# vedantsawal/Cost-and-Carbon-Aware-Kubernetes-Autoscaler

Measured on AMD Instinct MI355X. Metric: policy-evaluated cluster-steps/sec, higher is better.
Workload: dtype int32+int64+f64; 1 GPU; config2: 1e5 clusters x 1 deployment x 1440 one-minute steps, HPA + peak/off-peak, 16-type catalog; scenarios_per_gpu=100000, steps_per_rollout=1440, mode=trajectory, schedule=lane-skewed (single deployment), trace_layout=wave-tiled [wave][T][lanes] (built by the first rollout), parallelism=scenario-sharded x1

## Files before the change

cost-and-carbon-aware-kubernetes-autoscaler_amd/csrc/d1_common.h:

```cpp
#pragma once
#include <hip/hip_runtime.h>
#include <stdint.h>

#include "../../include/ccka.h"
#include "kparams.h"

namespace ccka {
namespace {

constexpr int WAVE = 64;

__device__ __forceinline__ int capbit1(int c) { return c == 0 ? CCKA_CAP_SPOT : CCKA_CAP_OD; }

template <class V>
__device__ __forceinline__ V opq(V v) {
  asm volatile("" : "+s"(v));
  return v;
}
#define GLOBAL_AS __attribute__((address_space(1)))
template <class V>
__device__ __forceinline__ GLOBAL_AS V* opq_ptr(V* v) {
  uint64_t x = (uint64_t)v;
  asm volatile("" : "+s"(x));
  return (GLOBAL_AS V*)x;
}

__device__ __forceinline__ int wmask(int window_s) {
  int m = 0;
#pragma unroll
  for (int k = 0; k < CCKA_HIST; ++k) m |= ((k + 1) * CCKA_STEP_SECONDS < window_s) ? (1 << k) : 0;
  return m;
}

template <int W = 4>
__device__ __forceinline__ void ring_push(uint32_t* r, int v) {
#pragma unroll
  for (int w = W - 1; w > 0; --w) r[w] = __builtin_amdgcn_alignbit(r[w], r[w - 1], 16);
  r[0] = (r[0] << 16) | ((uint32_t)v & 0xFFFFu);
}
template <int W>
__device__ __forceinline__ void ring_push4(uint32_t* r, int v) {
#pragma unroll
  for (int w = W - 1; w > 1; --w) r[w] = r[w - 2];
  r[1] = r[0] = ((uint32_t)v & 0xFFFFu) * 0x10001u;
}

typedef short short2v __attribute__((ext_vector_type(2)));
__device__ __forceinline__ short2v as_s2(uint32_t x) { return __builtin_bit_cast(short2v, x); }
__device__ __forceinline__ uint32_t bfi(uint32_t m, uint32_t a, uint32_t b) { return (m & a) | (~m & b); }

__device__ __forceinline__ int fdiv_nb(int a, int b, float rb, bool& bad) {
  int q = (int)((float)a * rb);
  const int r = (int)((uint32_t)a - (uint32_t)q * (uint32_t)b);
  q += (r >= b ? 1 : 0) - (r < 0 ? 1 : 0);
  bad = bad || (uint32_t)q >= (1u << 20) || (uint32_t)b >= (1u << 30);
  return q;
}

constexpr int D1_NOSTORE = 0x7FFFFFF0;
__device__ __forceinline__ void d1_store_rec(__amdgpu_buffer_rsrc_t r, int voff, const int4& v) {
  typedef int i32x4 __attribute__((ext_vector_type(4)));
  const i32x4 x = {v.x, v.y, v.z, v.w};
  __builtin_amdgcn_raw_buffer_store_b128(x, r, voff, 0, 0);
}

#define CONST_AS __attribute__((address_space(4)))
__device__ __forceinline__ int2 d1_tload(const GLOBAL_AS int2* ptr) {
  const uint64_t a = (uint64_t)ptr;
  const int alo = (int)(uint32_t)a, ahi = (int)(uint32_t)(a >> 32);
  const int me = (int)(threadIdx.x & (WAVE - 1));
  uint64_t m = __ballot(1);
  int ox = 0, oy = 0;
  while (m) {
    int l[4];
#pragma unroll
    for (int k = 0; k < 4; ++k) {
      l[k] = m ? __ffsll((long long)m) - 1 : l[0];
      m &= m - 1;
    }
    uint64_t v[4];
#pragma unroll
    for (int k = 0; k < 4; ++k) {
      const uint64_t ak = (uint64_t)(uint32_t)__builtin_amdgcn_readlane(alo, l[k]) |
                          (uint64_t)(uint32_t)__builtin_amdgcn_readlane(ahi, l[k]) << 32;
      v[k] = *(const CONST_AS uint64_t*)ak;
    }
#pragma unroll
    for (int k = 0; k < 4; ++k) {
      ox = me == l[k] ? (int)(uint32_t)v[k] : ox;
      oy = me == l[k] ? (int)(uint32_t)(v[k] >> 32) : oy;
    }
  }
  return make_int2(ox, oy);
}

}
}
```

cost-and-carbon-aware-kubernetes-autoscaler_amd/csrc/rollout_d1.hip:

```cpp
#include <hip/hip_runtime.h>
#include <stdint.h>

#include "../../include/ccka.h"
#include "d1_common.h"
#include "kparams.h"

#pragma clang fp contract(off)

namespace ccka {

namespace {

struct Best {
  double s;
  int k;
  int info;
  int price;
};

__device__ __forceinline__ bool better(double s2, int k2, double s, int k) {
  return s2 < s || (s2 == s && k2 < k);
}

__device__ __forceinline__ void take_if_better(Best& a, const Best& b) {
// ... 187 lines not shown
          bool G3 = false, bool KEDA = false>
__global__ void __launch_bounds__(256, OCC) rollout_d1_kernel(D1Params p) {
  static_assert(NSUB == 1 || (NSUB == 4 && BDEF), "15 s sync: lean default path");
  static_assert(!KEDA || (BDEF && NSUB == 1 && !DRIFT), "KEDA: default behavior, one decision per step");
  static_assert(HE == 8 || (HE == 4 && NSUB == 1 && BDEF), "4-record ring: default behavior, one decision per step");
  static_assert(!G3 || (DRIFT && MAXP == 2), "G3: the DRIFT instantiation, two pools");
  constexpr int HW = NSUB == 1 ? HE / 2 : 10;
  constexpr int JR = NSUB == 1 ? HE : 5;
  uint64_t st_acc[12] = {0, 0, 0, 0, 0, 0, 0, 0, 0, 0, 0, 0};
  uint64_t st_last = STAMPS ? __builtin_amdgcn_s_memtime() : 0;
  extern __shared__ __attribute__((aligned(16))) int4 s_acc[];
  for (int x = threadIdx.x; x < p.K; x += blockDim.x) {
    const long long idle = p.acc[x * 3 + 0];
    s_acc[x] = make_int4((int)(idle & 0xffffffffLL), (int)(idle >> 32), (int)p.acc[x * 3 + 1], (int)p.acc[x * 3 + 2]);
  }
  const bool ldt = p.lds_tab;
  const uint32_t tab_off = ((uint32_t)p.K * 16u + 255u) / 256u * 256u + (blockDim.x / WAVE) * (uint32_t)D1_RING_BYTES;
  const int n_pr = p.R * 24 * p.K * p.Z * 2;
  const int n_pr8 = (n_pr + 1) & ~1;
  int* const s_price = reinterpret_cast<int*>(reinterpret_cast<char*>(s_acc) + tab_off);
  double* const s_ci = reinterpret_cast<double*>(s_price + n_pr8);
  int* const s_jtab = reinterpret_cast<int*>(s_ci + p.R * 24);
  if (ldt) {
    for (int x = threadIdx.x; x < n_pr; x += blockDim.x) s_price[x] = p.price[x];
    for (int x = threadIdx.x; x < p.R * 24; x += blockDim.x) s_ci[x] = p.ci_gpwmin[x];
    for (int x = threadIdx.x; x < p.R * 24 * p.NZI * 3; x += blockDim.x) s_jtab[x] = p.jtab[x];
  }
  __syncthreads();
  const int lane = threadIdx.x & (WAVE - 1);
  const int64_t wv = (int64_t)xcd_block(blockIdx.x, gridDim.x) * (blockDim.x / WAVE) + (threadIdx.x / WAVE);
  const int64_t i = wv * p.lpw + lane;
  if (lane >= p.lpw || i >= p.N) return;

  const int r = p.region ? (int)p.region[i] : 0;
  const int target = KEDA ? 1 : (p.target ? (int)p.target[i] : p.target0);
  const int mx = KEDA ? opq(p.k_max) : (p.maxr ? (int)p.maxr[i] : p.maxr0);
  const int dwin = (!KEDA && p.down_stab) ? (int)p.down_stab[i] : p.dstab0;
  const int nd = min(NSUB == 1 ? __popc(wmask(dwin)) : (dwin > 15 ? (dwin - 1) / 15 : 0), 2 * HW);
  const int dnmask = NSUB == 1 ? wmask(dwin) : 0;
  const int reset_ca = p.reset_ca ? (int)p.reset_ca[i] : p.reset_ca0;
  const int pswitch = p.pswitch ? (int)p.pswitch[i] : p.pswitch0;
  const int wi = p.wci ? (int)p.wci[i] : 0;
  const uint32_t capsel = p.cap_sel ? (uint32_t)p.cap_sel[i] : (uint32_t)p.capsel0;
  const int minr = KEDA ? max(opq(p.k_min), 1) : opq(p.minr), req = opq(p.req_cpu), limit = opq(p.limit);
  const int kthr = KEDA ? opq(p.k_thr) : 1, kact = KEDA ? opq(p.k_act) : 0, kcds = KEDA ? opq(p.k_cds) : 0;
  const bool kmin0 = KEDA && opq(p.k_min) == 0;
  const float rkthr = __builtin_amdgcn_rcpf((float)kthr);
  int ulo = max(0, (int)floor(p.tol_lo * (double)target) - 2);
  while ((double)ulo / (double)target < p.tol_lo) ++ulo;
  int uhi = (int)floor(p.tol_hi * (double)target) + 2;
  while ((double)uhi / (double)target > p.tol_hi) --uhi;
  const float rtarget = __builtin_amdgcn_rcpf((float)target);

  const int NP = opq(p.NP), NZI = opq(p.NZI), NW = opq(p.NW), JT = opq(p.JT);
  const int maxn = opq(p.maxn), ablate = CCKA_ABLATE_BUILD ? opq(p.ablate) : 0, pdb_member = opq(p.pdb_member);
  const int pdb_pct = opq(p.pdb_pct), slo_util = opq(p.slo_util), delay = opq(p.delay);
  const int base_nodes = opq(p.base_nodes), base_type = opq(p.base_type);
  const int K = opq(p.K), Z = opq(p.Z), T = opq(p.T);
  const int ps = opq(p.peak_start) % 1440, pe = opq(p.peak_end) % 1440;
  const int ps_raw = opq(p.peak_start), pe_raw = opq(p.peak_end);
  const int sm0 = opq(p.start_minute) % 1440;
  const long long base_nw = opq(p.base_nw);
  const GLOBAL_AS int32_t* const price = opq_ptr(p.price);
  const GLOBAL_AS double* const ci_gpwmin = opq_ptr(p.ci_gpwmin);
  const GLOBAL_AS int2* const table = opq_ptr(p.table);
  const GLOBAL_AS int2* const table2 = opq_ptr(p.table2);
  const int drift_on = opq(p.drift_on), replace = opq(p.replace), multi = G3 ? opq(p.multi) : 0;
  const GLOBAL_AS int32_t* const jtab = opq_ptr(p.jtab);
  GLOBAL_AS int4* const traj = opq_ptr(reinterpret_cast<int4*>(p.traj));
  const D1Rule rup = [&] { if constexpr (BDEF) return d1_default_rule(true); else return opq_rule(p.up); }();
  const D1Rule rdn = [&] { if constexpr (BDEF) return d1_default_rule(false); else return opq_rule(p.dn); }();
  int budget[MAXP];
#pragma unroll
  for (int q = 0; q < MAXP; ++q) budget[q] = opq(p.budget[q]);

  int ppol[MAXP], pcas[MAXP], pzi[MAXP], pJ[MAXP];
  uint32_t pcm[MAXP], pmask[MAXP];
#pragma unroll
  for (int q = 0; q < MAXP; ++q) {
    ppol[q] = 0; pcas[q] = 0; pzi[q] = -1; pcm[q] = 0; pJ[q] = 0; pmask[q] = 0;
    if (q < NP) {
#pragma unroll
      for (int s = 0; s < 2; ++s) {
        const D1Patch& x = p.patch[q][s];
        if (x.policy) ppol[q] = x.policy;
        if (x.cas >= 0) pcas[q] = s == 1 ? (reset_ca + CCKA_STEP_SECONDS - 1) / CCKA_STEP_SECONDS : x.cas;
        if (x.zi >= 0) pzi[q] = x.zi;
        if (x.cm) pcm[q] = (uint32_t)x.cm;
      }
    }
  }

  auto cas_of = [&](uint32_t info) {
    const int m1 = -(int)(info >> 13 & 1u), m2 = -(int)(info >> 14 & 1u);
    const int lo = pcas[0] ^ ((pcas[0] ^ pcas[MAXP > 1 ? 1 : 0]) & m1);
    if constexpr (MAXP <= 2) {
      return lo;
    } else {
      const int hi = pcas[2] ^ ((pcas[2] ^ pcas[3]) & m1);
      return lo ^ ((lo ^ hi) & m2);
    }
  };
  auto casc = [](int c) { return min(c, 0xFFFF); };

  uint32_t sinfo[MAXN];
  int sready[MAXN], slc[MAXN], scas[MAXN], spods[MAXN], sprice[MAXN], scap[MAXN];
  uint32_t sdyn[MAXN];
  int salloc[MAXN];
  int sallocr[MAXN];
#pragma unroll
  for (int n = 0; n < MAXN; ++n) {
    sinfo[n] = 0; sready[n] = 0; slc[n] = 0; scas[n] = 0; spods[n] = 0; sprice[n] = 0; scap[n] = 0;
    sdyn[n] = 0; salloc[n] = 0; sallocr[n] = 0;
  }
  uint32_t used = 0, rdy = 0, cmask = 0;
  auto dyn_of = [&](int n) -> uint32_t {
    if constexpr (G3) return (uint32_t)s_acc[sinfo[n] & 1023u].z;
    else return sdyn[n];
  };
  auto alloc_of = [&](int n) -> int {
    if constexpr (G3) return s_acc[sinfo[n] & 1023u].w;
    else return salloc[n];
  };
  constexpr bool kAllocR = NSUB == 1 && !G3;
  auto alloc_ready = [&](int n) -> uint32_t {
    if constexpr (kAllocR) return (uint32_t)sallocr[n];
    else return (rdy >> n & 1u) ? (uint32_t)alloc_of(n) : 0u;
  };
  auto cas_slot = [&](int n) -> int {
    if constexpr (G3) return casc(cas_of(sinfo[n]));
    else return scas[n];
  };
  uint32_t dmask = 0, srcm = 0, repm = 0;
  auto taint = [&]() -> uint32_t { return DRIFT ? (srcm | repm) : 0u; };
  auto od_slots = [&]() {
    uint32_t m = 0;
#pragma unroll
    for (int n = MAXN - 1; n >= 0; --n) m = 2 * m + (sinfo[n] >> 12 & 1u);
    return m & used;
  };
  const uint32_t slot_mask = maxn >= 32 ? 0xFFFFFFFFu : ((1u << maxn) - 1u);

  int replicas = p.replicas0, placed = 0, rpods = 0;
  uint32_t hdn[HW], hup[4], hdel[4] = {0, 0, 0, 0};
  uint32_t dn16[HW];
#pragma unroll
  for (int w = 0; w < 4; ++w) hup[w] = 0x7FFF7FFFu;
#pragma unroll
  for (int w = 0; w < HW; ++w) {
    hdn[w] = 0x80008000u;
    dn16[w] = (2 * w < nd ? 0xFFFFu : 0u) | (2 * w + 1 < nd ? 0xFFFF0000u : 0u);
  }
  int next_ready = 0x7fffffff, nsp = 0, nod = 0;
  int kcd = kcds, q_klo = 0, q_khi = -1, kb_cur = -1;
  bool q_kcd = false;
  bool k_act_step = false;
  auto keda_band = [&](int cur) {
    if (!KEDA || cur == kb_cur) return;
    kb_cur = cur;
    if (cur <= 0) { q_klo = 0; q_khi = -1; return; }
    const double D = (double)kthr * (double)cur;
    long long lo = max((long long)floor(p.tol_lo * D) - 2, -1LL);
    while ((double)lo / D < p.tol_lo) ++lo;
    long long hi = (long long)floor(p.tol_hi * D) + 2;
    while ((double)hi / D > p.tol_hi) --hi;
    q_klo = (int)min(lo, 0x7fffffffLL);
    q_khi = (int)min(hi, 0x7ffffffeLL);
  };
  keda_band(p.replicas0);
  int Ffree = 0;
  int minscap = 0x7fffffff;
  int profile = -1, hour = -1;
  long long cost = 0, burn = 0, base_price = 0;
  int pend_min = 0;
  long long energy_nw = 0, e_hour = 0, Isum = 0;
  double gco2 = 0.0, ci_min = 0.0;
  int slo = 0, nmin_spot = 0, nmin_od = 0, launches = 0, deletions = 0, peak_nodes = 0;
  uint32_t last_choice = 0xFFFFFFFFu, hash = 2166136261u;

  unsigned long long Ssum = 0;
  float Rmax = 0.f;
  float q_rbd = 0.f, q_rbc = 0.f, q_rbp = 0.f;
  bool q_peak = false;
  int q_rcap = 0;
  int q_hold = -0x40000000;
  (void)dnmask;
  const int wl = NSUB == 1 ? nd : max(0, (nd - (NSUB - 1)) / NSUB);
  const int wr = NSUB == 1 ? nd : (nd + NSUB - 1) / NSUB;
  int q_ulim = 0, q_pge = 0, q_slo = 0, q_usat = 0, q_w0 = 0, q_w1 = 0, q_pendv = 0, q_nodes = 0;
  float q_hbp = 0.f;
  uint32_t usum = 0;
  bool q_met = false;

  auto refresh_J = [&](int rh) {
#pragma unroll
    for (int q = 0; q < MAXP; ++q) {
      const uint32_t cm = pcm[q] & capsel;
      const int64_t ji = ((int64_t)rh * NZI + pzi[q]) * 3 + (cm - 1);
      pJ[q] = (q < NP && cm && pzi[q] >= 0) ? (ldt ? s_jtab[ji] : jtab[ji]) : 0;
    }
  };

  struct HpaOut {
    int util, proposal, desired;
    bool ran, hpa_path;
  };
  auto behave = [&](int proposal, int cur) -> int {
    int upr = proposal, dnr = proposal;
    if (rup.stab_mask) {
      short2v a = as_s2(bfi((uint32_t)rup.stab16[0], hup[0], 0x7FFF7FFFu));
#pragma unroll
      for (int w = 1; w < 4; ++w)
        a = __builtin_elementwise_min(a, as_s2(bfi((uint32_t)rup.stab16[w], hup[w], 0x7FFF7FFFu)));
      upr = min(upr, min((int)a.x, (int)a.y));
    }
    {
      short2v a = as_s2(bfi(dn16[0], hdn[0], 0x80008000u));
#pragma unroll
      for (int w = 1; w < HW; ++w) a = __builtin_elementwise_max(a, as_s2(bfi(dn16[w], hdn[w], 0x80008000u)));
      dnr = max(dnr, max((int)a.x, (int)a.y));
    }
    const int rc = min(max(cur, upr), dnr);
    int lo = minr, hi = mx;
    if constexpr (BDEF) {
      hi = rc > cur ? min(hi, max(2 * cur, cur + 4)) : hi;
      lo = rc < cur ? max(lo, 0) : lo;
    } else {
      if (proposal != cur) {
        if (rc > cur) hi = min(hi, max(rate_limit1(rup, true, cur, hdel), cur));
        else if (rc < cur) lo = max(lo, min(rate_limit1(rdn, false, cur, hdel), cur));
      }
    }
    return rc < lo ? lo : (rc > hi ? hi : rc);
  };
  auto hpa_eval = [&](int L, int cur, int ready, float rbd, float rbc) -> HpaOut {
    HpaOut o;
    const bool metric = cur <= mx && cur >= minr && ready > 0 && !(cur == 0 && minr != 0);
    int util = 0, proposal = cur;
    {
      const int rcapv = ready * limit;
      const int usage = (limit > 0 && rcapv < L) ? rcapv : L;
      const int a = usage * 100;
      const int dreq = ready * req;
      const int dcur = cur * req;
      bool slow = usage < 0 || usage > 21474836;
      util = fdiv_nb(a, dreq, rbd, slow);
      int nu = 0;
      if (cur > ready) nu = fdiv_nb(a, dcur, rbc, slow);
      if (__builtin_expect(metric && slow, 0))
        util = (int)(((long long)usage * 100) / ((long long)ready * req));
      const bool unready_up = cur > ready && util > target;
      int u = util, base = ready;
// ... 121 lines not shown
  }();
  const int32_t* lp = p.load_w ? p.load_w + wtb * T + lane
                               : p.load + (p.trace_mod > 0 ? (p.first_id + i) % p.trace_mod : i);
  const long long lsl = opq(p.load_w ? (long long)p.lpw : (long long)p.NL);
  const uint32_t ring_off = (uint32_t)__builtin_amdgcn_readfirstlane(
      (int)(((uint32_t)p.K * 16u + 255u) / 256u * 256u + (threadIdx.x / WAVE) * (uint32_t)D1_RING_BYTES));
  const uint32_t ring_lds = (uint32_t)(uintptr_t)s_acc + ring_off;
  const int* const ring = reinterpret_cast<const int*>(reinterpret_cast<const char*>(s_acc) + ring_off);
  constexpr int rsw = WAVE, rbn = D1_RB;
  auto rrow = [&](int x) { return x & (D1_RB - 1); };
  auto ridx = [&](int r) { return r * rsw + lane; };
  auto rnext = [&](int r, int q) { return (r + q) & (D1_RB - 1); };
  int tf = 0;
  int tfr = 0;
  const int32_t* lpf = lp;
  auto tf_adv = [&]() {
    ++tf;
    ++tfr;
    if (tfr == rbn) tfr = 0;
    lpf += lsl;
  };
  {
    const int n0 = min(T, D1_VMN + 4 * D1_S);
    while (tf < n0) {
      d1_dma_row(lpf, (uint32_t)__builtin_amdgcn_readfirstlane((int)(ring_lds + (uint32_t)tfr * (uint32_t)(rsw * 4))));
      tf_adv();
    }
    d1_wait_all();
  }
  int t_rdy = tf;
  bool pf_ok = false;
  bool qadv = true;
  int Lpf[D1_S];
#pragma unroll
  for (int q = 0; q < D1_S; ++q) Lpf[q] = 0;
  const int64_t w0 = wtb;
  const int wlanes = (int)min((int64_t)p.lpw, p.N - w0);
  const __amdgpu_buffer_rsrc_t trs = __builtin_amdgcn_make_buffer_rsrc(
      traj ? (void*)(reinterpret_cast<int4*>(p.traj) + w0 * T) : (void*)p.load, 0, traj ? wlanes * T * 16 : 0,
      0x00020000);
  const int lb = lane * T * 16;

  for (int it = 0;; ++it) {
    const bool live = t < T;
    if (__ballot(live) == 0) break;
    d1_wait_rows();
    t_rdy = max(t_rdy, tf - D1_VMN);
    const uint64_t sb = __ballot(stall);
    if constexpr (STAMPS) st_acc[9] += 1;
    if (sb != 0 && (it % D1_K == D1_K - 1 || !qadv)) {
      __builtin_amdgcn_s_setprio(0);
      if constexpr (STAMPS) { st_acc[10] += 1; st_acc[11] += __popcll(sb); }
      const bool ev = stall;
      int L = 0, minute = 0, rh = 0, pd = 0, step_last_type = 0xFFFF;
      int4 rec;
      uint32_t flags = 0;
      bool g_acted = false, hchg = false, jchg = false;
      uint32_t emp_e = 0, weou_e = 0;
      HpaOut hp{};
      if (ev) {
        stall = false;
        const int tr = rrow(t);
        L = ring[ridx(tr)];
        if constexpr (BDEF) {
          const int kq = min(t - tq, wr);
          if (kq > 0) {
            const int cur16 = min(replicas, D1_REC_SAT);
            int us[JR], rv[JR];
            bool anylow = false;
#pragma unroll
            for (int j = 0; j < JR; ++j) {
              us[j] = KEDA ? ring[ridx(rnext(tr, rbn - 1 - j))] : min(ring[ridx(rnext(tr, rbn - 1 - j))], q_rcap);
              rv[j] = q_met ? cur16 : (int)0x8000;
              anylow |= (j < kq) & q_met & (us[j] < q_pge);
            }
            if (KEDA && anylow) {
#pragma unroll
              for (int j = 0; j < JR; ++j) {
                bool sl = false;
                const bool low = (j < kq) & q_met & (us[j] < q_pge);
                const int q = fdiv_nb(max(us[j], 0), kthr, rkthr, sl);
                rv[j] = low ? min(q + (q * kthr != us[j] ? 1 : 0), D1_REC_SAT) : rv[j];
              }
            } else if (anylow) {
              const int dreq = rpods * req;
              const float rbd = __builtin_amdgcn_rcpf((float)dreq);
              bool anyex = false;
#pragma unroll
              for (int j = 0; j < JR; ++j) {
                bool sl = false;
                const bool low = (j < kq) & q_met & (us[j] < q_pge);
                const int util = fdiv_nb(us[j] * 100, dreq, rbd, sl);
                const int x = (int)__umul24((uint32_t)util, (uint32_t)rpods);
                const int q = fdiv_nb(x, target, rtarget, sl);
                const bool ex = x == q * target;
                anyex |= low & ex;
                rv[j] = low ? min(q + (ex ? 0 : 1), D1_REC_SAT) : rv[j];
                us[j] = (low & ex) ? util : -1;
              }
              if (__builtin_expect(anyex, 0)) {
#pragma unroll
                for (int j = 0; j < JR; ++j)
                  if (us[j] >= 0)
                    rv[j] = min((int)ceil(((double)us[j] / (double)target) * (double)rpods), D1_REC_SAT);
              }
            }
#pragma unroll
            for (int j = JR - 1; j >= 0; --j)
              if (j < kq) {
                if constexpr (NSUB == 1) ring_push<HW>(hdn, rv[j]);
                else ring_push4<HW>(hdn, rv[j]);
              }
          }
        }
        flush(t);
        minute = (sm0 + t) % 1440;
        const int h = minute / 60;
        rh = r * 24 + h;
        if (h != hour) {
          if (hour >= 0) {
            gco2 += (double)e_hour * (ci_min * 1e-9);
            energy_nw += e_hour;
          }
          e_hour = 0;
          hour = h;
          hchg = true;
        }
      }
      D1_STAMP(2);
      if (ev) {
        if (t >= next_ready) {
          next_ready = 0x7fffffff;
#pragma unroll
          for (int n = 0; n < MAXN; ++n) {
            if ((used & ~rdy) >> n & 1u) {
              if (sready[n] <= t) {
                rdy |= 1u << n;
                rpods += spods[n];
                sallocr[n] = salloc[n];
                if ((cmask & ~taint()) >> n & 1u) Ffree += scap[n] - spods[n];
              }
              else next_ready = min(next_ready, sready[n]);
            }
          }
        }
        const bool in_win = ps_raw <= pe_raw ? (minute >= ps_raw && minute < pe_raw)
                                             : (minute >= ps_raw || minute < pe_raw);
        const bool peak = pswitch && in_win;
        const int prof = peak ? CCKA_PROFILE_PEAK : CCKA_PROFILE_OFFPEAK;
        if (peak) flags |= 1u;
        q_peak = peak;
        if (prof != profile) {
          profile = prof;
          int pold[MAXP];
#pragma unroll
          for (int q = 0; q < MAXP; ++q) pold[q] = pcas[q];
#pragma unroll
          for (int q = 0; q < MAXP; ++q) {
            if (q >= NP) break;
            const D1Patch& x = p.patch[q][prof + 1];
            if (x.policy) ppol[q] = x.policy;
            if (x.cas >= 0) pcas[q] = x.cas;
            if (x.zi >= 0) pzi[q] = x.zi;
            if (x.cm) pcm[q] = (uint32_t)x.cm;
          }
#pragma unroll
          for (int n = 0; n < MAXN; ++n)
            if (used >> n & 1u) {
              const int c = casc(cas_of(sinfo[n]));
              if constexpr (G3) {
                const int m1 = -(int)(sinfo[n] >> 13 & 1u);
                const int o = pold[0] ^ ((pold[0] ^ pold[MAXP > 1 ? 1 : 0]) & m1);
                slc[n] += c - casc(o);
              } else {
                slc[n] += c - scas[n];
              }
              scas[n] = c;
            }
          jchg = true;
          if (DRIFT && drift_on) {
            uint32_t dm = 0;
#pragma unroll
            for (int n = 0; n < MAXN; ++n) {
              const uint32_t x = sinfo[n];
              uint32_t zm = 0, cm = 0;
#pragma unroll
              for (int q = 0; q < MAXP; ++q)
                if ((int)(x >> 13 & 3u) == q) { zm = pzi[q] >= 0 ? p.zml[pzi[q]] : 0u; cm = pcm[q]; }
              const bool drifted = !(zm >> (x >> 10 & 3u) & 1u) || !(cm & capbit1((int)(x >> 12 & 1u)));
              dm |= ((used >> n & 1u) && drifted ? 1u : 0u) << n;
            }
            dmask = dm;
          }
        }

      }
      D1_STAMP(3);
      if (ev) {
#pragma unroll
        for (int sub = 0; sub < NSUB; ++sub) {
          const int cur = replicas;
          if constexpr (KEDA) hp = keda_eval(L, cur, t);
          else
            hp = hpa_eval(L, cur, rpods, __builtin_amdgcn_rcpf((float)(rpods * req)),
                          __builtin_amdgcn_rcpf((float)(cur * req)));
          hpa_commit(hp, cur);
          replicas = hp.desired;
        }

        if (placed > replicas) {
          int excess = placed - replicas;
          placed = replicas;
#pragma unroll
          for (int pass = 0; pass < 2; ++pass) {
            const uint32_t m = pass == 0 ? (used & ~rdy) : rdy;
            if (!m || excess <= 0) continue;
            int removed = 0, removed_c = 0;
#pragma unroll
            for (int n = MAXN - 1; n >= 0; --n) {
              const int k = (m >> n & 1u) ? min(spods[n], excess) : 0;
              spods[n] -= k;
              excess -= k;
              removed += k;
              if (pass == 1) removed_c += ((cmask & ~taint()) >> n & 1u) ? k : 0;
              slc[n] = k > 0 ? t + cas_slot(n) : slc[n];
            }
            if (pass == 1) { rpods -= removed; Ffree += removed_c; }
          }
        }
        pd = replicas - placed;
        if (pd > 0) {
#pragma unroll
          for (int pass = 0; pass < 2; ++pass) {
            const uint32_t m = (pass == 0 ? rdy : (used & ~rdy)) & cmask & ~taint();
            if (!m || pd <= 0) continue;
            int added = 0;
#pragma unroll
            for (int n = 0; n < MAXN; ++n) {
              const int fr = (m >> n & 1u) ? scap[n] - spods[n] : 0;
              const int k = min(fr, pd);
              spods[n] += k;
              pd -= k;
              added += k;
              slc[n] = k > 0 ? t + cas_slot(n) : slc[n];
            }
            placed += added;
            if (pass == 0) { rpods += added; Ffree -= added; }
          }
        }
      }
      D1_STAMP(4);
      if (ev) {
        if (hchg) {
          const int64_t toff = (int64_t)rh * K * Z * 2;
          const GLOBAL_AS int32_t* tile = price + toff;
          const int* stile = s_price + toff;
          ci_min = ldt ? s_ci[rh] : ci_gpwmin[rh];
          base_price = (long long)base_nodes * (ldt ? stile[(base_type * Z) * 2 + 1] : tile[(base_type * Z) * 2 + 1]);
          burn = 0;
          int np[MAXN];
#pragma unroll
          for (int n = 0; n < MAXN; ++n) {
            const uint32_t x = sinfo[n];
            const int e = ((int)(x & 1023u) * Z + (int)(x >> 10 & 3u)) * 2 + (int)(x >> 12 & 1u);
            np[n] = ldt ? stile[e] : tile[e];
          }
#pragma unroll
          for (int n = 0; n < MAXN; ++n) {
            if (used >> n & 1u) {
              sprice[n] = np[n];
              burn += np[n];
            }
          }
        }
        if (hchg || jchg) refresh_J(rh);
        {
          uint32_t fm = ~used & slot_mask;
          if (pd > 0 && fm && !ablated(ablate, 2)) {
            int q = -1, J = 0, zq = 0, cq = 0;
            uint32_t cm = 0;
#pragma unroll
            for (int qq = MAXP - 1; qq >= 0; --qq) {
              const uint32_t c = pcm[qq] & capsel;
              if (qq < NP && c && pJ[qq] > 0) { q = qq; J = pJ[qq]; cm = c; zq = pzi[qq]; cq = pcas[qq]; }
            }
            if (q >= 0) {
              const GLOBAL_AS int2* row = table + ((((int64_t)rh * NZI + zq) * 3 + (cm - 1)) * NW + wi) * JT;
              while (pd > 0 && fm) {
                const int slot = __ffs((int)fm) - 1;
                fm &= fm - 1;
                const int k = min(J, pd);
                const int2 e = d1_tload(row + k);
                const int info = e.y, price = e.x;
                const int bk = info & 1023, bz = info >> 10 & 3, bc = info >> 12 & 1, cap1 = info >> 16;
                const int rs = t + delay;
                const int4 ac = s_acc[bk];
#pragma unroll
                for (int n = 0; n < MAXN; ++n) {
                  if (n == slot) {
                    sinfo[n] = (uint32_t)(bk | bz << 10 | bc << 12 | q << 13);
                    sready[n] = rs;
                    slc[n] = t + casc(cq);
                    scas[n] = casc(cq);
                    spods[n] = k;
                    sprice[n] = price;
                    scap[n] = cap1;
                    sdyn[n] = (uint32_t)ac.z;
                    salloc[n] = ac.w;
                    sallocr[n] = delay == 0 ? ac.w : 0;
                  }
                }
                const uint32_t bit = 1u << slot;
                used |= bit;
                if (capbit1(bc) & capsel) cmask |= bit;
#pragma unroll
                for (int qq = 0; qq < MAXP; ++qq) if (qq == q) pmask[qq] |= bit;
                placed += k;
                minscap = min(minscap, cap1);
                Isum += ((long long)ac.y << 32) | (unsigned)ac.x;
                if (delay == 0) {
                  rdy |= bit;
                  rpods += k;
                  if (cmask & bit) Ffree += cap1 - k;
                }
                else next_ready = min(next_ready, rs);
                if (bc == 0) nsp++; else nod++;
                burn += price;
                launches++;
                last_choice = (uint32_t)bk | (uint32_t)bz << 12 | (uint32_t)bc << 14 | (uint32_t)q << 16;
                hash = (hash ^ last_choice) * 16777619u;
                step_last_type = bk;
                flags |= 2u;
                pd -= k;
              }
            }
          }
        }

      }
      D1_STAMP(5);
      if (ev) {
        uint32_t elig = 0, emp = 0;
#pragma unroll
        for (int n = MAXN - 1; n >= 0; --n) {
          elig = 2 * elig + (slc[n] <= t ? 1u : 0u);
          emp = 2 * emp + (spods[n] == 0 ? 1u : 0u);
        }
        elig &= rdy;
        emp &= used;
        uint32_t weou = 0;
#pragma unroll
        for (int q = 0; q < MAXP; ++q)
          if (q < NP && ppol[q] == CCKA_WHEN_EMPTY_OR_UNDERUTILIZED) weou |= pmask[q];
        weou_e = weou;
        const uint32_t g2c = (DRIFT && replace) ? (weou & od_slots() & ~emp & ~srcm) : 0u;
        const uint32_t g3c = (DRIFT && G3 && multi) ? (weou & ~emp & ~taint()) : 0u;
        const uint32_t gate = elig & (emp | (Ffree >= minscap ? weou : (weou & ~cmask)) | g2c | g3c);
        const uint32_t tkm = DRIFT ? (repm & rdy) : 0u;
        const uint32_t dwork = DRIFT ? (dmask & rdy & ~srcm) : 0u;
        if ((gate || tkm || dwork) && !ablated(ablate, 1)) {
          bool any_del = false;
          auto ffree_now = [&]() {
            int f = 0;
            const uint32_t m = rdy & cmask & ~taint();
#pragma unroll
            for (int n = 0; n < MAXN; ++n) f += (m >> n & 1u) ? scap[n] - spods[n] : 0;
            Ffree = f;
          };
          auto masks_now = [&]() {
            uint32_t el = 0, em = 0;
#pragma unroll
            for (int n = MAXN - 1; n >= 0; --n) {
              el = 2 * el + (slc[n] <= t ? 1u : 0u);
              em = 2 * em + (spods[n] == 0 ? 1u : 0u);
            }
            elig = el & rdy;
            emp = em & used;
          };
          auto drop_slot = [&](int b) {
            uint32_t binfo = 0;
            int bprice = 0;
#pragma unroll
            for (int n = 0; n < MAXN; ++n)
              if (n == b) {
                binfo = sinfo[n];
                bprice = sprice[n];
                sallocr[n] = 0;
                spods[n] = 0;
                sinfo[n] = 0;
              }
            if ((binfo >> 12 & 1u) == 0) nsp--; else nod--;
            burn -= bprice;
            const int4 ac = s_acc[binfo & 1023u];
            Isum -= ((long long)ac.y << 32) | (unsigned)ac.x;
            const uint32_t nb = ~(1u << b);
            used &= nb; rdy &= nb; cmask &= nb; dmask &= nb; srcm &= nb; repm &= nb;
#pragma unroll
            for (int qq = 0; qq < MAXP; ++qq) pmask[qq] &= nb;
            deletions++;
            any_del = true;
          };
          if constexpr (DRIFT) {
            if (tkm) {
              uint32_t tk = tkm;
              while (tk) {
                const int m = __ffs((int)tk) - 1;
                tk &= tk - 1;
                uint32_t xm = 0;
                int capm = 0, podm = 0;
#pragma unroll
                for (int n = 0; n < MAXN; ++n)
                  if (n == m) { xm = sinfo[n]; sinfo[n] = xm & 0xFFFFu; capm = scap[n]; podm = spods[n]; }
                const bool okc = (capbit1((int)(xm >> 12 & 1u)) & capsel) != 0;
                uint32_t sm = xm >> 16 & 0xFFu;
                int got = 0;
                while (sm) {
                  const int src = __ffs((int)sm) - 1;
                  sm &= sm - 1;
                  int sp = 0;
#pragma unroll
                  for (int n = 0; n < MAXN; ++n) sp = n == src ? spods[n] : sp;
                  const int k = okc ? min(capm - podm - got, sp) : 0;
                  got += k;
                  rpods -= sp - k;
                  placed -= sp - k;
                  drop_slot(src);
                }
#pragma unroll
                for (int n = 0; n < MAXN; ++n)
                  if (n == m) { spods[n] += got; slc[n] = t + cas_slot(n); }
                repm &= ~(1u << m);
                flags |= 4u;
              }
              ffree_now();
              masks_now();
            }
          }
          int allowed = 0x7fffffff;
          if (pdb_pct >= 0) {
            const int rdyp = pdb_member ? rpods : 0, reps = pdb_member ? replicas : 0;
            allowed = max(rdyp - (int)(((uint32_t)(pdb_pct * reps) + 99u) / 100u), 0);
          }
#pragma unroll
          for (int q = 0; q < MAXP; ++q) {
            if (q >= NP) break;
            const int npool = __popc(pmask[q]);
            if (npool == 0) continue;
            const int qbudget = (budget[q] * npool + 99) / 100;
            const bool weou_q = ppol[q] == CCKA_WHEN_EMPTY_OR_UNDERUTILIZED;
            int deleted = 0;
            if constexpr (DRIFT) {
              uint32_t dc = dmask & rdy & ~srcm & pmask[q];
              bool acted = false;
              while (dc && deleted < qbudget) {
                const int best = __ffs((int)dc) - 1;
                dc &= dc - 1;
                int bp = 0;
#pragma unroll
                for (int n = 0; n < MAXN; ++n) bp = n == best ? spods[n] : bp;
                const int pdbp = pdb_member ? bp : 0;
                if (pdbp > allowed) continue;
                acted = true;
                const uint32_t recv = rdy & ~dmask & ~taint() & cmask;
                int need = bp;
#pragma unroll
                for (int n = 0; n < MAXN; ++n) {
                  const int fr = (recv >> n & 1u) ? scap[n] - spods[n] : 0;
                  const int k = min(fr, need);
                  spods[n] += k;
                  need -= k;
                  slc[n] = k > 0 ? t + cas_slot(n) : slc[n];
                }
                const uint32_t fr = ~used & slot_mask;
                int2 e = make_int2(0, -1);
                uint32_t cmq = 0;
                int cq = 0;
                if (need > 0 && fr) {
                  int J = 0, zq = -1;
#pragma unroll
                  for (int qq = 0; qq < MAXP; ++qq)
                    if (qq == q) { J = pJ[qq]; zq = pzi[qq]; cmq = pcm[qq] & capsel; cq = pcas[qq]; }
                  if (cmq && zq >= 0 && need <= J)
                    e = d1_tload(table + ((((int64_t)rh * NZI + zq) * 3 + (cmq - 1)) * NW + wi) * JT + need);
                }
                if (e.y >= 0 && need > 0) {
                  const int info = e.y, price = e.x;
                  const int bk = info & 1023, bz = info >> 10 & 3, bc = info >> 12 & 1, cap1 = info >> 16;
                  const int slot = __ffs((int)fr) - 1;
                  const int rs = t + delay;
                  const int4 ac = s_acc[bk];
#pragma unroll
                  for (int n = 0; n < MAXN; ++n) {
                    if (n == slot) {
                      sinfo[n] = (uint32_t)(bk | bz << 10 | bc << 12 | q << 13) | (1u << (16 + best));
                      sready[n] = rs;
                      slc[n] = t + casc(cq);
                      scas[n] = casc(cq);
                      spods[n] = 0;
                      sprice[n] = price;
                      scap[n] = cap1;
                      sdyn[n] = (uint32_t)ac.z;
                      salloc[n] = ac.w;
                      sallocr[n] = delay == 0 ? ac.w : 0;
                    }
                    if (n == best) spods[n] = need;
                  }
                  const uint32_t bit = 1u << slot;
                  used |= bit;
                  if (capbit1(bc) & capsel) cmask |= bit;
#pragma unroll
                  for (int qq = 0; qq < MAXP; ++qq) if (qq == q) pmask[qq] |= bit;
                  if (delay == 0) rdy |= bit;
                  else next_ready = min(next_ready, rs);
                  minscap = min(minscap, cap1);
                  Isum += ((long long)ac.y << 32) | (unsigned)ac.x;
                  if (bc == 0) nsp++; else nod++;
                  burn += price;
                  launches++;
                  last_choice = (uint32_t)bk | (uint32_t)bz << 12 | (uint32_t)bc << 14 | (uint32_t)q << 16;
                  hash = (hash ^ last_choice) * 16777619u;
                  step_last_type = bk;
                  srcm |= 1u << best;
                  repm |= bit;
                  flags |= 2u | 16u | 32u;
                } else {
                  rpods -= need;
                  placed -= need;
                  drop_slot(best);
                  flags |= 4u | 16u;
                }
                allowed -= pdbp;
                deleted++;
              }
              if (acted) {
                g_acted = true;
                ffree_now();
// ... 101 lines not shown
                  uint32_t cmq = 0;
                  int zq = -1, cq = 0;
#pragma unroll
                  for (int qq = 0; qq < MAXP; ++qq)
                    if (qq == q) { zq = pzi[qq]; cmq = pcm[qq] & capsel; cq = pcas[qq]; }
                  const uint32_t fr = ~used & slot_mask;
                  int lo = 1, hi = nc - 1, bestk = 0, mid = 0;
                  while (true) {
                    int k;
                    bool commit = false;
                    if (lo <= hi) { mid = (lo + hi) / 2; k = mid + 1; }
                    else if (bestk) { k = bestk; commit = true; }
                    else break;
                    uint32_t set = 0;
                    for (int r = 0; r < k; ++r) set |= 1u << (ord >> (4 * r) & 15u);
                    int tp[MAXN];
                    int pdbp = 0;
                    long long psum = 0;
                    uint32_t anyod = 0;
#pragma unroll
                    for (int n = 0; n < MAXN; ++n) {
                      tp[n] = spods[n];
                      const bool in = set >> n & 1u;
                      pdbp += in ? spods[n] : 0;
                      psum += in ? sprice[n] : 0;
                      anyod |= in ? (sinfo[n] >> 12 & 1u) : 0u;
                    }
                    bool ok = !(pdb_member && pdbp > allowed);
                    uint32_t touched = 0;
                    const uint32_t recv = rdy & ~tn & ~set & cmask;
                    for (int r = 0; r < k; ++r) {
                      const int c = (int)(ord >> (4 * r) & 15u);
                      int need = 0;
#pragma unroll
                      for (int n = 0; n < MAXN; ++n) need = n == c ? tp[n] : need;
#pragma unroll
                      for (int m = 0; m < MAXN; ++m) {
                        const int f = (recv >> m & 1u) ? scap[m] - tp[m] : 0;
                        const int kk = min(f, need);
                        tp[m] += kk;
                        need -= kk;
                        touched |= (kk > 0 ? 1u : 0u) << m;
                      }
#pragma unroll
                      for (int n = 0; n < MAXN; ++n) tp[n] = n == c ? need : tp[n];
                    }
                    int sp = 0;
#pragma unroll
                    for (int n = 0; n < MAXN; ++n) sp += (set >> n & 1u) ? tp[n] : 0;
                    int2 e = make_int2(0, -1);
                    if (ok && sp > 0) {
                      const uint32_t cm = anyod ? cmq : (cmq & ~(uint32_t)CCKA_CAP_SPOT);
                      ok = cm != 0 && fr != 0 && zq >= 0 && sp < JT;
                      if (ok) e = d1_tload(table2 + (((int64_t)rh * NZI + zq) * 3 + (cm - 1)) * JT + sp);
                      ok = ok && e.y >= 0 && (long long)e.x < psum;
                    }
                    if (!commit) {
                      if (ok) { bestk = k; lo = mid + 1; }
                      else hi = mid - 1;
                      continue;
                    }
                    uint32_t srcmask = 0;
#pragma unroll
                    for (int n = 0; n < MAXN; ++n) {
                      spods[n] = tp[n];
                      slc[n] = (touched >> n & 1u) ? t + cas_slot(n) : slc[n];
                      srcmask |= ((set >> n & 1u) && tp[n] > 0 ? 1u : 0u) << n;
                    }
                    uint32_t gone = set & ~srcmask;
                    while (gone) {
                      const int n = __ffs((int)gone) - 1;
                      gone &= gone - 1;
                      drop_slot(n);
                      flags |= 4u;
                    }
                    if (sp > 0) {
                      const int info = e.y, prc = e.x;
                      const int bk = info & 1023, bz = info >> 10 & 3, bc = info >> 12 & 1, cap1 = info >> 16;
                      const int slot = __ffs((int)fr) - 1;
                      const int rs = t + delay;
                      const int4 ac = s_acc[bk];
#pragma unroll
                      for (int n = 0; n < MAXN; ++n) {
                        if (n == slot) {
                          sinfo[n] = (uint32_t)(bk | bz << 10 | bc << 12 | q << 13) | (srcmask << 16);
                          sready[n] = rs;
                          slc[n] = t + casc(cq);
                          scas[n] = casc(cq);
                          spods[n] = 0;
                          sprice[n] = prc;
                          scap[n] = cap1;
                          sdyn[n] = (uint32_t)ac.z;
                          salloc[n] = ac.w;
                          sallocr[n] = delay == 0 ? ac.w : 0;
                        }
                      }
                      const uint32_t bit = 1u << slot;
                      used |= bit;
                      if (capbit1(bc) & capsel) cmask |= bit;
#pragma unroll
                      for (int qq = 0; qq < MAXP; ++qq) if (qq == q) pmask[qq] |= bit;
                      if (delay == 0) rdy |= bit;
                      else next_ready = min(next_ready, rs);
                      minscap = min(minscap, cap1);
                      Isum += ((long long)ac.y << 32) | (unsigned)ac.x;
                      if (bc == 0) nsp++; else nod++;
                      burn += prc;
                      launches++;
                      last_choice = (uint32_t)bk | (uint32_t)bz << 12 | (uint32_t)bc << 14 | (uint32_t)q << 16;
                      hash = (hash ^ last_choice) * 16777619u;
                      step_last_type = bk;
                      srcm |= srcmask;
                      repm |= bit;
                      flags |= 2u | 32u;
                    }
                    flags |= 64u;
                    if (pdb_member) allowed -= pdbp;
                    deleted += k;
                    any_del = true;
                    g_acted = true;
                    g3_acted = true;
                    ffree_now();
                    masks_now();
                    break;
                  }
                }
              }
            }
            if constexpr (DRIFT) {
              if (replace && weou_q && !g3_acted && deleted < qbudget) {
                uint32_t c2 = elig & pmask[q] & od_slots() & ~emp & ~srcm;
                while (c2) {
                  unsigned long long bkey = ~0ull;
#pragma unroll
                  for (int n = 0; n < MAXN; ++n) {
                    const unsigned long long key = (unsigned long long)spods[n] << 36 |
                                                   (unsigned long long)(0x7fffffff - sprice[n]) << 4 | (unsigned)n;
                    bkey = ((c2 >> n & 1u) && key < bkey) ? key : bkey;
                  }
                  const int best = (int)(bkey & 15u), bp = (int)(bkey >> 36);
                  const int bpr = 0x7fffffff - (int)((bkey >> 4) & 0x7fffffffull);
                  const uint32_t fr = ~used & slot_mask;
                  if (!fr) break;
                  uint32_t cmq = 0;
                  int zq = -1, cq = 0;
#pragma unroll
                  for (int qq = 0; qq < MAXP; ++qq)
                    if (qq == q) { zq = pzi[qq]; cmq = pcm[qq] & capsel; cq = pcas[qq]; }
                  int2 e = make_int2(0, -1);
                  if (!(pdb_member && bp > allowed) && cmq && zq >= 0)
                    e = d1_tload(table2 + (((int64_t)rh * NZI + zq) * 3 + (cmq - 1)) * JT + bp);
                  if (e.y < 0 || e.x >= bpr) {
                    c2 &= ~(1u << best);
                    continue;
                  }
                  const int info = e.y, prc = e.x;
                  const int bk = info & 1023, bz = info >> 10 & 3, bc = info >> 12 & 1, cap1 = info >> 16;
                  const int slot = __ffs((int)fr) - 1;
                  const int rs = t + delay;
                  const int4 ac = s_acc[bk];
#pragma unroll
                  for (int n = 0; n < MAXN; ++n) {
                    if (n == slot) {
                      sinfo[n] = (uint32_t)(bk | bz << 10 | bc << 12 | q << 13) | (1u << (16 + best));
                      sready[n] = rs;
                      slc[n] = t + casc(cq);
                      scas[n] = casc(cq);
                      spods[n] = 0;
                      sprice[n] = prc;
                      scap[n] = cap1;
                      sdyn[n] = (uint32_t)ac.z;
                      salloc[n] = ac.w;
                      sallocr[n] = delay == 0 ? ac.w : 0;
                    }
                  }
                  const uint32_t bit = 1u << slot;
                  used |= bit;
                  if (capbit1(bc) & capsel) cmask |= bit;
#pragma unroll
                  for (int qq = 0; qq < MAXP; ++qq) if (qq == q) pmask[qq] |= bit;
                  if (delay == 0) rdy |= bit;
                  else next_ready = min(next_ready, rs);
                  minscap = min(minscap, cap1);
                  Isum += ((long long)ac.y << 32) | (unsigned)ac.x;
                  if (bc == 0) nsp++; else nod++;
                  burn += prc;
                  launches++;
                  last_choice = (uint32_t)bk | (uint32_t)bz << 12 | (uint32_t)bc << 14 | (uint32_t)q << 16;
                  hash = (hash ^ last_choice) * 16777619u;
                  step_last_type = bk;
                  srcm |= 1u << best;
                  repm |= bit;
                  flags |= 2u | 32u;
                  deleted++;
                  g_acted = true;
                  break;
                }
              }
            }
          }
          if (any_del) {
            g_acted = true;
            minscap = 0x7fffffff;
#pragma unroll
// ... 69 lines not shown
              uge = min(uge, max(us, 0));
              lim = umin(uhi + 1, dreq);
            }
            pge = umin(uge, dreq);
            ulim = replicas >= mx ? UQ : lim;
            if (!pend) slo_thr = umin(max(slo_util + 1, 0), dreq);
          } else if (dnm == replicas) {
            ulim = UQ;
          }
          if constexpr (KEDA) {
            met = false;
            ulim = 0;
            pge = UQ;
            slo_thr = pend ? 0 : UQ;
            q_kcd = false;
            if (replicas == 0) {
              ulim = (int)min(max((long long)kact + 1, 0LL), (long long)UQ);
              pge = 0;
            } else if (replicas >= minr && replicas <= mx) {
              met = true;
              q_kcd = kmin0;
              keda_band(replicas);
              ulim = replicas >= mx ? UQ : (int)min((long long)q_khi + 1, (long long)UQ);
              const long long lc = (long long)(replicas - 1) * kthr + 1;
              pge = (int)max(0LL, min(min((long long)q_klo, lc), (long long)UQ));
            }
            q_met = met;
          }
          q_ulim = ulim;
          q_pge = pge;
          q_slo = slo_thr;
          q_rbp = rpods > 0 ? __builtin_amdgcn_rcpf((float)rpods) : 0.f;
          q_hbp = 0.5f * q_rbp;
          q_usat = Rmax > 0.f ? (int)fminf(0.9999f * __builtin_amdgcn_rcpf(Rmax), 1073741824.0f) - 1 : 0x7fffffff;
          q_pendv = replicas - rpods;
          q_nodes = (nsp & 0xFFFF) | nod << 16;
          q_w0 = 0xFFFF | (int)((q_peak ? 1u : 0u) << 16);
          q_w1 = q_w0 | (8 << 16);
        } else {
          q_rbd = __builtin_amdgcn_rcpf((float)(rpods * req));
          q_rbc = __builtin_amdgcn_rcpf((float)(replicas * req));
        }
        if constexpr (BDEF) {
          int hit = -0x40000000;
#pragma unroll
          for (int k = 2 * HW - 1; k >= 0; --k) {
            const int e = (int)(short)(hdn[k >> 1] >> (16 * (k & 1)));
            hit = e >= replicas ? t - k / NSUB : hit;
          }
          q_hold = replicas <= minr ? 0x3fffffff : hit + wl;
          if (!q_met) q_hold = 0x3fffffff;
        }
        {
          const int th = t + 60 - minute % 60;
          int nx = min(next_ready, th);
          if (pswitch) {
            if (t >= npb) {
              const int dps = (ps - minute + 1439) % 1440 + 1, dpe = (pe - minute + 1439) % 1440 + 1;
              npb = t + min(dps, dpe);
            }
            nx = min(nx, npb);
          }
          const uint32_t gm = rdy & (emp_e | (Ffree >= minscap ? weou_e : (weou_e & ~cmask)) |
                                     ((DRIFT && replace) ? (weou_e & od_slots() & ~emp_e & ~srcm) : 0u) |
                                     ((DRIFT && G3 && multi) ? (weou_e & ~emp_e & ~taint()) : 0u));
#pragma unroll
          for (int n = 0; n < MAXN; ++n) nx = ((gm >> n & 1u) && slc[n] > t) ? min(nx, slc[n]) : nx;
          if (g_acted || ablated(ablate, 15)) nx = t + 1;
          nxt = nx;
        }
      }
      if (ev) {
        d1_store_rec(trs, lb + t * 16, rec);
        ++t;
      }
      pf_ok = pf_ok && !ev;
      D1_STAMP(7);
    }
    __builtin_amdgcn_s_setprio(D1_PRIO_HI);
    if (tf < T) {
      if (__ballot(t < T && t < tf + D1_S - rbn + D1_BACK) == 0) {
        const int n1 = min(T, tf + D1_S);
        while (tf < n1) {
          d1_dma_row(lpf, (uint32_t)__builtin_amdgcn_readfirstlane((int)(ring_lds + (uint32_t)tfr * (uint32_t)(rsw * 4))));
          tf_adv();
        }
        if (tf == T) {
          d1_wait_all();
          t_rdy = T;
        }
      }
    }
    bool adv = false;
    if (!pf_ok) {
      const int tr = rrow(t);
#pragma unroll
      for (int q = 0; q < D1_S; ++q) Lpf[q] = ring[ridx(rnext(tr, q))];
    }

    D1_STAMP(8);
    const int tlim = min(T, t_rdy);
#pragma unroll
    for (int sub = 0; sub < D1_S; ++sub) {
    if constexpr (BDEF) {
        const int L = Lpf[sub];
        const int usage = min(L, q_rcap);
        const int cv = KEDA ? L : usage;
        const bool ge = cv >= q_pge;
        bool ok = (t < nxt) & ((uint32_t)cv < (uint32_t)q_ulim) & (ge | (t <= q_hold));
        const bool kac = KEDA && L > kact;
        if constexpr (KEDA) ok = ok & (!q_kcd | kac | (t < kcd));
// ... 178 lines not shown
```

Before: 76.04 billion cluster-steps/s.

## Pack cold scalar params into one SGPR and reload rare args from kernarg

Packs several small per-launch parameters (NZI, NW, Z, PDB fields) into one bit-packed scalar decoded with s_bfe, and reloads rarely used pointers and fields (jtab, price, ci, peak bounds, NP) from the kernarg segment when needed instead of keeping them live. The per-step minute/hour computation with modulo and divide is replaced by incremental hour and day counters, and several q<NP guards are dropped. The aim is to cut scalar register pressure and per-step integer division in the hot loop. It risks extra scalar loads on cold paths, and the dropped NP guards rely on unused patch slots being zero. Index math narrows from 64-bit to 32-bit in places.

Measured after the change: 76.54 billion cluster-steps/s (median of 6 runs). Within noise of the previous version (+0.7%).

```diff
diff --git a/cost-and-carbon-aware-kubernetes-autoscaler_amd/csrc/d1_common.h b/cost-and-carbon-aware-kubernetes-autoscaler_amd/csrc/d1_common.h
--- a/cost-and-carbon-aware-kubernetes-autoscaler_amd/csrc/d1_common.h
+++ b/cost-and-carbon-aware-kubernetes-autoscaler_amd/csrc/d1_common.h
@@ -1,5 +1,6 @@
 #pragma once
 #include <hip/hip_runtime.h>
+#include <stddef.h>
 #include <stdint.h>
 
 #include "../../include/ccka.h"
@@ -23,6 +24,22 @@
   uint64_t x = (uint64_t)v;
   asm volatile("" : "+s"(x));
   return (GLOBAL_AS V*)x;
+}
+
+#define CONST_AS __attribute__((address_space(4)))
+template <class V>
+__device__ __forceinline__ V cold_arg(size_t off) {
+  uint64_t a = (uint64_t)__builtin_amdgcn_kernarg_segment_ptr();
+  asm volatile("" : "+s"(a));
+  return *(const CONST_AS V*)(a + off);
+}
+#define D1_COLD(field) cold_arg<decltype(D1Params::field)>(offsetof(D1Params, field))
+
+template <uint32_t SPEC>
+__device__ __forceinline__ int pk_get(uint32_t pk) {
+  int v;
+  asm volatile("s_bfe_u32 %0, %1, %2" : "=s"(v) : "s"(pk), "n"(SPEC) : "scc");
+  return v;
 }
 
 __device__ __forceinline__ int wmask(int window_s) {
@@ -64,7 +81,6 @@
   __builtin_amdgcn_raw_buffer_store_b128(x, r, voff, 0, 0);
 }
 
-#define CONST_AS __attribute__((address_space(4)))
 __device__ __forceinline__ int2 d1_tload(const GLOBAL_AS int2* ptr) {
   const uint64_t a = (uint64_t)ptr;
   const int alo = (int)(uint32_t)a, ahi = (int)(uint32_t)(a >> 32);
diff --git a/cost-and-carbon-aware-kubernetes-autoscaler_amd/csrc/rollout_d1.hip b/cost-and-carbon-aware-kubernetes-autoscaler_amd/csrc/rollout_d1.hip
--- a/cost-and-carbon-aware-kubernetes-autoscaler_amd/csrc/rollout_d1.hip
+++ b/cost-and-carbon-aware-kubernetes-autoscaler_amd/csrc/rollout_d1.hip
@@ -263,21 +263,20 @@
   while ((double)uhi / (double)target > p.tol_hi) --uhi;
   const float rtarget = __builtin_amdgcn_rcpf((float)target);
 
-  const int NP = opq(p.NP), NZI = opq(p.NZI), NW = opq(p.NW), JT = opq(p.JT);
-  const int maxn = opq(p.maxn), ablate = CCKA_ABLATE_BUILD ? opq(p.ablate) : 0, pdb_member = opq(p.pdb_member);
-  const int pdb_pct = opq(p.pdb_pct), slo_util = opq(p.slo_util), delay = opq(p.delay);
-  const int base_nodes = opq(p.base_nodes), base_type = opq(p.base_type);
-  const int K = opq(p.K), Z = opq(p.Z), T = opq(p.T);
-  const int ps = opq(p.peak_start) % 1440, pe = opq(p.peak_end) % 1440;
+  const uint32_t pk = opq((uint32_t)p.NZI | (uint32_t)p.NW << 4 | (uint32_t)p.Z << 8 |
+                          (uint32_t)(p.pdb_member != 0) << 12 | (uint32_t)(p.pdb_pct + 1) << 16);
+  constexpr uint32_t PK_NZI = 0 | 4 << 16, PK_NW = 4 | 4 << 16, PK_Z = 8 | 4 << 16, PK_PDBM = 12 | 1 << 16,
+                     PK_PDBP1 = 16 | 8 << 16;
+  const int JT = opq(p.JT);
+  const int maxn = opq(p.maxn), ablate = CCKA_ABLATE_BUILD ? opq(p.ablate) : 0;
+  const int slo_util = opq(p.slo_util), delay = opq(p.delay);
+  const int base_nodes = opq(p.base_nodes), T = opq(p.T);
+  const int tile_n = opq(p.K * p.Z * 2), base_off = opq(p.base_type * p.Z * 2 + 1);
   const int ps_raw = opq(p.peak_start), pe_raw = opq(p.peak_end);
-  const int sm0 = opq(p.start_minute) % 1440;
   const long long base_nw = opq(p.base_nw);
-  const GLOBAL_AS int32_t* const price = opq_ptr(p.price);
-  const GLOBAL_AS double* const ci_gpwmin = opq_ptr(p.ci_gpwmin);
   const GLOBAL_AS int2* const table = opq_ptr(p.table);
   const GLOBAL_AS int2* const table2 = opq_ptr(p.table2);
   const int drift_on = opq(p.drift_on), replace = opq(p.replace), multi = G3 ? opq(p.multi) : 0;
-  const GLOBAL_AS int32_t* const jtab = opq_ptr(p.jtab);
   GLOBAL_AS int4* const traj = opq_ptr(reinterpret_cast<int4*>(p.traj));
   const D1Rule rup = [&] { if constexpr (BDEF) return d1_default_rule(true); else return opq_rule(p.up); }();
   const D1Rule rdn = [&] { if constexpr (BDEF) return d1_default_rule(false); else return opq_rule(p.dn); }();
@@ -290,7 +289,7 @@
 #pragma unroll
   for (int q = 0; q < MAXP; ++q) {
     ppol[q] = 0; pcas[q] = 0; pzi[q] = -1; pcm[q] = 0; pJ[q] = 0; pmask[q] = 0;
-    if (q < NP) {
+    if (q < p.NP) {
 #pragma unroll
       for (int s = 0; s < 2; ++s) {
         const D1Patch& x = p.patch[q][s];
@@ -381,7 +380,10 @@
   keda_band(p.replicas0);
   int Ffree = 0;
   int minscap = 0x7fffffff;
-  int profile = -1, hour = -1;
+  int profile = -1;
+  const int sm0 = p.start_minute % 1440;
+  const int rh_end = r * 24 + 24;
+  int rh = r * 24 + sm0 / 60, th = 60 - sm0 % 60, moff = sm0;
   long long cost = 0, burn = 0, base_price = 0;
   int pend_min = 0;
   long long energy_nw = 0, e_hour = 0, Isum = 0;
@@ -404,11 +406,12 @@
   bool q_met = false;
 
   auto refresh_J = [&](int rh) {
+    const int NZI = pk_get<PK_NZI>(pk);
 #pragma unroll
     for (int q = 0; q < MAXP; ++q) {
       const uint32_t cm = pcm[q] & capsel;
-      const int64_t ji = ((int64_t)rh * NZI + pzi[q]) * 3 + (cm - 1);
-      pJ[q] = (q < NP && cm && pzi[q] >= 0) ? (ldt ? s_jtab[ji] : jtab[ji]) : 0;
+      const int ji = (rh * NZI + pzi[q]) * 3 + (int)(cm - 1);
+      pJ[q] = (cm && pzi[q] >= 0) ? (ldt ? s_jtab[ji] : ((const GLOBAL_AS int32_t*)D1_COLD(jtab))[ji]) : 0;
     }
   };
 
@@ -636,7 +639,7 @@
       __builtin_amdgcn_s_setprio(0);
       if constexpr (STAMPS) { st_acc[10] += 1; st_acc[11] += __popcll(sb); }
       const bool ev = stall;
-      int L = 0, minute = 0, rh = 0, pd = 0, step_last_type = 0xFFFF;
+      int L = 0, minute = 0, pd = 0, step_last_type = 0xFFFF;
       int4 rec;
       uint32_t flags = 0;
       bool g_acted = false, hchg = false, jchg = false;
@@ -698,16 +701,19 @@
           }
         }
         flush(t);
-        minute = (sm0 + t) % 1440;
-        const int h = minute / 60;
-        rh = r * 24 + h;
-        if (h != hour) {
-          if (hour >= 0) {
+        const bool hend = t >= th;
+        th += hend ? 60 : 0;
+        rh += hend ? 1 : 0;
+        const bool dend = rh == rh_end;
+        rh -= dend ? 24 : 0;
+        moff -= dend ? 1440 : 0;
+        minute = t + moff;
+        if (hend || t == 0) {
+          if (t != 0) {
             gco2 += (double)e_hour * (ci_min * 1e-9);
             energy_nw += e_hour;
           }
           e_hour = 0;
-          hour = h;
           hchg = true;
         }
       }
@@ -741,7 +747,7 @@
           for (int q = 0; q < MAXP; ++q) pold[q] = pcas[q];
 #pragma unroll
           for (int q = 0; q < MAXP; ++q) {
-            if (q >= NP) break;
+            if (q >= D1_COLD(NP)) break;
             const D1Patch& x = p.patch[q][prof + 1];
             if (x.policy) ppol[q] = x.policy;
             if (x.cas >= 0) pcas[q] = x.cas;
@@ -836,11 +842,12 @@
       D1_STAMP(4);
       if (ev) {
         if (hchg) {
-          const int64_t toff = (int64_t)rh * K * Z * 2;
-          const GLOBAL_AS int32_t* tile = price + toff;
+          const int Z = pk_get<PK_Z>(pk);
+          const int toff = rh * tile_n;
+          const GLOBAL_AS int32_t* tile = ldt ? nullptr : (const GLOBAL_AS int32_t*)D1_COLD(price) + toff;
           const int* stile = s_price + toff;
-          ci_min = ldt ? s_ci[rh] : ci_gpwmin[rh];
-          base_price = (long long)base_nodes * (ldt ? stile[(base_type * Z) * 2 + 1] : tile[(base_type * Z) * 2 + 1]);
+          ci_min = ldt ? s_ci[rh] : ((const GLOBAL_AS double*)D1_COLD(ci_gpwmin))[rh];
+          base_price = (long long)base_nodes * (ldt ? stile[base_off] : tile[base_off]);
           burn = 0;
           int np[MAXN];
 #pragma unroll
@@ -866,10 +873,12 @@
 #pragma unroll
             for (int qq = MAXP - 1; qq >= 0; --qq) {
               const uint32_t c = pcm[qq] & capsel;
-              if (qq < NP && c && pJ[qq] > 0) { q = qq; J = pJ[qq]; cm = c; zq = pzi[qq]; cq = pcas[qq]; }
+              if (c && pJ[qq] > 0) { q = qq; J = pJ[qq]; cm = c; zq = pzi[qq]; cq = pcas[qq]; }
             }
             if (q >= 0) {
-              const GLOBAL_AS int2* row = table + ((((int64_t)rh * NZI + zq) * 3 + (cm - 1)) * NW + wi) * JT;
+              const int NZI = pk_get<PK_NZI>(pk), NW = pk_get<PK_NW>(pk);
+              const int key = ((rh * NZI + zq) * 3 + (int)(cm - 1)) * NW + wi;
+              const GLOBAL_AS int2* row = table + (int64_t)key * JT;
               while (pd > 0 && fm) {
                 const int slot = __ffs((int)fm) - 1;
                 fm &= fm - 1;
@@ -935,7 +944,7 @@
         uint32_t weou = 0;
 #pragma unroll
         for (int q = 0; q < MAXP; ++q)
-          if (q < NP && ppol[q] == CCKA_WHEN_EMPTY_OR_UNDERUTILIZED) weou |= pmask[q];
+          if (ppol[q] == CCKA_WHEN_EMPTY_OR_UNDERUTILIZED) weou |= pmask[q];
         weou_e = weou;
         const uint32_t g2c = (DRIFT && replace) ? (weou & od_slots() & ~emp & ~srcm) : 0u;
         const uint32_t g3c = (DRIFT && G3 && multi) ? (weou & ~emp & ~taint()) : 0u;
@@ -944,6 +953,7 @@
         const uint32_t dwork = DRIFT ? (dmask & rdy & ~srcm) : 0u;
         if ((gate || tkm || dwork) && !ablated(ablate, 1)) {
           bool any_del = false;
+          const int pdb_member = pk_get<PK_PDBM>(pk), pdb_pct = pk_get<PK_PDBP1>(pk) - 1;
           auto ffree_now = [&]() {
             int f = 0;
             const uint32_t m = rdy & cmask & ~taint();
@@ -1027,7 +1037,6 @@
           }
 #pragma unroll
           for (int q = 0; q < MAXP; ++q) {
-            if (q >= NP) break;
             const int npool = __popc(pmask[q]);
             if (npool == 0) continue;
             const int qbudget = (budget[q] * npool + 99) / 100;
@@ -1065,7 +1074,8 @@
                   for (int qq = 0; qq < MAXP; ++qq)
                     if (qq == q) { J = pJ[qq]; zq = pzi[qq]; cmq = pcm[qq] & capsel; cq = pcas[qq]; }
                   if (cmq && zq >= 0 && need <= J)
-                    e = d1_tload(table + ((((int64_t)rh * NZI + zq) * 3 + (cmq - 1)) * NW + wi) * JT + need);
+                    e = d1_tload(table + ((((int64_t)rh * pk_get<PK_NZI>(pk) + zq) * 3 + (cmq - 1)) * pk_get<PK_NW>(pk) + wi) *
+                                             JT + need);
                 }
                 if (e.y >= 0 && need > 0) {
                   const int info = e.y, price = e.x;
@@ -1273,7 +1283,8 @@
                     if (ok && sp > 0) {
                       const uint32_t cm = anyod ? cmq : (cmq & ~(uint32_t)CCKA_CAP_SPOT);
                       ok = cm != 0 && fr != 0 && zq >= 0 && sp < JT;
-                      if (ok) e = d1_tload(table2 + (((int64_t)rh * NZI + zq) * 3 + (cm - 1)) * JT + sp);
+                      if (ok)
+                        e = d1_tload(table2 + (((int64_t)rh * pk_get<PK_NZI>(pk) + zq) * 3 + (cm - 1)) * JT + sp);
                       ok = ok && e.y >= 0 && (long long)e.x < psum;
                     }
                     if (!commit) {
@@ -1370,7 +1381,7 @@
                     if (qq == q) { zq = pzi[qq]; cmq = pcm[qq] & capsel; cq = pcas[qq]; }
                   int2 e = make_int2(0, -1);
                   if (!(pdb_member && bp > allowed) && cmq && zq >= 0)
-                    e = d1_tload(table2 + (((int64_t)rh * NZI + zq) * 3 + (cmq - 1)) * JT + bp);
+                    e = d1_tload(table2 + (((int64_t)rh * pk_get<PK_NZI>(pk) + zq) * 3 + (cmq - 1)) * JT + bp);
                   if (e.y < 0 || e.x >= bpr) {
                     c2 &= ~(1u << best);
                     continue;
@@ -1546,11 +1557,13 @@
           if (!q_met) q_hold = 0x3fffffff;
         }
         {
-          const int th = t + 60 - minute % 60;
           int nx = min(next_ready, th);
           if (pswitch) {
             if (t >= npb) {
-              const int dps = (ps - minute + 1439) % 1440 + 1, dpe = (pe - minute + 1439) % 1440 + 1;
+              const int ps = D1_COLD(peak_start) % 1440, pe = D1_COLD(peak_end) % 1440;
+              int dps = ps - minute, dpe = pe - minute;
+              dps += dps <= 0 ? 1440 : 0;
+              dpe += dpe <= 0 ? 1440 : 0;
               npb = t + min(dps, dpe);
             }
             nx = min(nx, npb);
```
